# jafarinia/snuffy

Hardware: AMD Instinct MI355X
Metric: slides/sec (higher is better)
Workload: dtype f32; 1 GPU; cfgB: MILNet eval forward, 1 bag/step/rank, N=32768 patches D=768 h=6 Lambda=200 (K=200) depth=1 relu mlp x4; parallelism=bag-parallel x1, bags_resident_per_rank=8, launch=hip graph replay, rccl_ranks=0

## Files before the change

snuffy_amd/csrc/gemm.hip:

```cpp
#include <stdlib.h>

#include "mfma.h"
#include "philox.h"

namespace {

struct GemmParams {
    const unsigned short* a;
    const unsigned short* w;
    const float* bias;
    void* c;
    int64_t lda, ldw, ldc;
    int m, n, k;
    int act;
    int tiles_m, tiles_n;
    unsigned long long* trace;
    const float* resid = nullptr;
    int64_t ldr = 0;
    unsigned int* split_cnt = nullptr;
    float* split_slab = nullptr;
    int split_cap = 0, split_rcap = 0;
    const unsigned short* gate = nullptr;
    int64_t ldg = 0;
    const float* colsum = nullptr;
// ... 384 lines not shown
    for (int i = 0; i < AHEAD; ++i) stage(cur, i, i);
    wait_vmcnt<(AHEAD - 1) * GL>();
    __builtin_amdgcn_s_barrier();
    __builtin_amdgcn_sched_barrier(0);
    if (wid >= 4) __builtin_amdgcn_s_barrier();

    int rb = 0, sb = AHEAD;
    bool after_epilogue = false;
    while (true) {
        const int next = tile + wgs_per_xcd;
        const bool has_next = next < t_hi;
        const Src nxt = tile_src(has_next ? next : tile);
        const bool full = (tile / P.tiles_n + 1) * BM <= P.m && (tile % P.tiles_n + 1) * BN <= P.n;
        for (int s = 0; s < ns; ++s) {
            if constexpr (EPI == 2)
                if (s == 0) preload_x(tile);
            read_frags(rb);
            if (s == ns - 1) load_bias(tile);
            const bool in_tile = s + AHEAD < ns;
            const int exist = has_next ? AHEAD : (ns - 1 - s < AHEAD ? ns - 1 - s : AHEAD);
            if (in_tile)
                stage(cur, s + AHEAD, sb);
            else if (has_next)
                stage(nxt, s + AHEAD - ns, sb);
            if (exist == AHEAD) {
                if (after_epilogue)
                    wait_vmcnt<(AHEAD - 1) * GL + MI * NST>();
                else
                    wait_vmcnt<(AHEAD - 1) * GL>();
            } else if (AHEAD == 3 && exist == 2) {
                wait_vmcnt<GL>();
            } else {
                wait_vmcnt<0>();
            }
            after_epilogue = false;
            rb = rb == NBUF - 1 ? 0 : rb + 1;
            sb = sb == NBUF - 1 ? 0 : sb + 1;
            barrier();
            if (s == 0)
                mma(std::true_type{});
            else
                mma(std::false_type{});
            barrier();
        }
        bias_landed();
#ifdef SNF_GEMM_NOSTORE
        if (false) {
#else
        if (full) {
#endif
            epilogue(tile, std::true_type{});
            after_epilogue = true;
        } else {
            epilogue(tile, std::false_type{});
            wait_vmcnt<0>();
        }
        if (!has_next) break;
        tile = next;
        cur = nxt;
    }
    if (wid < 4) __builtin_amdgcn_s_barrier();
}

template <int ACT, int OUT, bool SPLIT = false, bool GATE = false, bool DROP = false>
__global__ __launch_bounds__(512, 2) void gemm_hl_kernel(GemmParams P) {
    static_assert(!GATE || (OUT == 3 && ACT == SNF_ACT_NONE && !SPLIT), "gemm_hl: the gated form writes an hl image, no activation, no split");
    static_assert(!DROP || (!GATE && (OUT == 1 || OUT == 3)), "gemm_hl: dropout goes with the fp32 and the hl-image outputs");
    constexpr int NI = 4, BN = 256;
    constexpr int ROWL = 128;
    constexpr int IMG = BM * ROWL;
    constexpr int STEP_BYTES = 2 * IMG;
    constexpr int NC = 4 * NI;
    constexpr bool LINE_STORES = (OUT == 1 || OUT == 3) && ACT != SNF_ACT_GELU && ACT != SNF_ACT_SELU;
    extern __shared__ __attribute__((aligned(16))) unsigned char smem[];

    const int lane = threadIdx.x & 63;
    const int wid = __builtin_amdgcn_readfirstlane(threadIdx.x >> 6);
    const int wr = wid >> 2, wc = wid & 3;
    const int ns_all = P.k / BKS;
    unsigned char* const scr = smem + 2 * STEP_BYTES + wid * 4096;

    const int ntiles = P.tiles_m * P.tiles_n;
    const int xcd = blockIdx.x & 7, wg_in_xcd = blockIdx.x >> 3, wgs_per_xcd = gridDim.x >> 3;
    if constexpr (!SPLIT) {
        if (P.split_cap >= 2 && blockIdx.x == 0) {
            for (int i = threadIdx.x; i < 8 * P.split_rcap; i += 512) P.split_cnt[i] = 0u;
            asm volatile("s_waitcnt vmcnt(0)" ::: "memory");
        }
    }
    int t_lo, t_hi;
    {
        const int q = ntiles >> 3, r = ntiles & 7;
        t_lo = xcd < r ? xcd * (q + 1) : r * (q + 1) + (xcd - r) * q;
        t_hi = t_lo + q + (xcd < r ? 1 : 0);
    }
    int sp_part = 0, sp_parts = 1, sp_slot = 0, sp_tile = -1;
    if (P.split_cap >= 2) {
        const int q_x = t_hi - t_lo, full_rounds = q_x / wgs_per_xcd, r = q_x - full_rounds * wgs_per_xcd;
        int sn = r > 0 ? wgs_per_xcd / r : 0;
        if (sn > P.split_cap) sn = P.split_cap;
        if (sn > ns_all / HL_SPLIT_MIN_STEPS) sn = ns_all / HL_SPLIT_MIN_STEPS;
        if (sn >= 2 && r <= P.split_rcap) {
            if constexpr (SPLIT) {
                if (wg_in_xcd < r * sn) {
                    const int jr = wg_in_xcd % r;
                    sp_tile = t_lo + full_rounds * wgs_per_xcd + jr;
                    sp_part = wg_in_xcd / r, sp_parts = sn, sp_slot = xcd * P.split_rcap + jr;
                }
            } else {
                t_hi = t_lo + full_rounds * wgs_per_xcd;
            }
        }
    }
    int tile = t_lo + wg_in_xcd;
    if constexpr (SPLIT) {
        tile = __builtin_amdgcn_readfirstlane(sp_tile);
        sp_part = __builtin_amdgcn_readfirstlane(sp_part), sp_parts = __builtin_amdgcn_readfirstlane(sp_parts);
        sp_slot = __builtin_amdgcn_readfirstlane(sp_slot);
        if (tile < 0) return;
        t_hi = tile + 1;
        asm volatile("" : "+s"(t_hi));
    } else {
        if (tile >= t_hi) return;
    }
    const int s_begin = SPLIT ? __builtin_amdgcn_readfirstlane(sp_part * ns_all / sp_parts) : 0;
    const int ns = SPLIT ? __builtin_amdgcn_readfirstlane((sp_part + 1) * ns_all / sp_parts) - s_begin : ns_all;
    const unsigned short* const a_base = P.a + (SPLIT ? s_begin * 64 : 0);
    const unsigned short* const w_base = P.w + (SPLIT ? s_begin * 64 : 0);

    struct Src {
        int a[4], w[4];
    };
    auto tile_src_mn = [&](int tm, int tn) __attribute__((always_inline)) -> Src {
        Src s;
        int ln = lane;
        asm volatile("" : "+v"(ln));
        const int c = ln & 7;
#pragma unroll
        for (int j = 0; j < 4; ++j) {
            const int row = (4 * wid + j) * 8 + (ln >> 3);
            int grow = tm * BM + row;
            if (grow > P.m - 1) grow = P.m - 1;
            s.a[j] = grow * (int)P.lda + ((c ^ ((row >> 1) & 7)) << 3);
            int wrow = tn * BN + row;
            if (wrow > P.n - 1) wrow = P.n - 1;
            s.w[j] = wrow * (int)P.ldw + ((c ^ (((row >> 1) & 1) | (((row >> 3) & 3) << 1))) << 3);
        }
        return s;
    };
    auto tile_src = [&](int tl) __attribute__((always_inline)) -> Src {
        const int tm = tl / P.tiles_n;
        return tile_src_mn(tm, tl - tm * P.tiles_n);
    };
    auto stage = [&](const Src& s, int kstep, int buf) __attribute__((always_inline)) {
#ifdef X3_NOSTAGE
        return;
#endif
        unsigned char* base = smem + buf * STEP_BYTES;
#pragma unroll
        for (int j = 0; j < 4; ++j) {
            __builtin_amdgcn_global_load_lds((glb_void*)(a_base + s.a[j] + kstep * 64), (lds_void*)(base + (4 * wid + j) * 1024), 16, 0, 0);
            __builtin_amdgcn_global_load_lds((glb_void*)(w_base + s.w[j] + kstep * 64), (lds_void*)(base + IMG + (4 * wid + j) * 1024), 16, 0, 0);
        }
    };

    const int fi = lane & 15, fg = lane >> 4;
    const int fa = (fi >> 1) & 7, fw = ((fi >> 1) & 1) | ((fi >> 2) << 1);
    const int xoff_h = (128 * wr + fi) * ROWL + ((fg ^ fa) << 4), xoff_l = (128 * wr + fi) * ROWL + (((4 + fg) ^ fa) << 4);
    const int wrow0 = IMG + (64 * wc + 8 * (fi >> 2) + (fi & 3)) * ROWL;
    const int woff_h = wrow0 + ((fg ^ fw) << 4), woff_l = wrow0 + (((4 + fg) ^ fw) << 4);

    f32x4 acc[8][NI];
    bf16x8 xf[8], wh[NI], wl[NI];
    f32x4 bv4[NC / 4];

    auto frag = [&](const unsigned char* p) __attribute__((always_inline)) -> bf16x8 {
#ifdef X3_NOREAD
        u32x4 z = {1u, 2u, 3u, (unsigned)lane};
        asm volatile("" : "+v"(z));
        return __builtin_bit_cast(bf16x8, z);
#endif
        return __builtin_bit_cast(bf16x8, *reinterpret_cast<const u32x4*>(p));
    };
#ifdef X3_NOMFMA
#define X3_MFMA(a, b, c) ([&]() { f32x4 t_ = (c); asm volatile("" : "+v"(t_) : "v"(a), "v"(b)); return t_; }())
#else
#define X3_MFMA(a, b, c) __builtin_amdgcn_mfma_f32_16x16x32_bf16(a, b, c, 0, 0, 0)
#endif
    auto load_bias = [&](int tl) __attribute__((always_inline)) {
#pragma unroll
        for (int c4 = 0; c4 < NC / 4; ++c4) bv4[c4] = f32x4{0.f, 0.f, 0.f, 0.f};
        if (P.bias) {
            const int tn = tl % P.tiles_n;
            const int n0 = tn * BN + 64 * wc + 8 * fg;
            const float* bp0 = P.bias + (n0 + 8 <= P.n ? n0 : 0);
            const float* bp1 = P.bias + (n0 + 40 <= P.n ? n0 + 32 : 0);
            asm volatile("global_load_dwordx4 %0, %1, off" : "=v"(bv4[0]) : "v"(bp0) : "memory");
            asm volatile("global_load_dwordx4 %0, %1, off offset:16" : "=v"(bv4[1]) : "v"(bp0) : "memory");
            asm volatile("global_load_dwordx4 %0, %1, off" : "=v"(bv4[2]) : "v"(bp1) : "memory");
            asm volatile("global_load_dwordx4 %0, %1, off offset:16" : "=v"(bv4[3]) : "v"(bp1) : "memory");
        }
    };
    auto bias_landed = [&]() __attribute__((always_inline)) {
#pragma unroll
        for (int c4 = 0; c4 < NC / 4; ++c4) asm volatile("" : "+v"(bv4[c4]));
    };
    auto epilogue = [&](int tl, auto full_t) __attribute__((always_inline)) {
        constexpr bool FULL = decltype(full_t)::value;
        const int tm = tl / P.tiles_n, tn = tl - tm * P.tiles_n;
        const int n0 = tn * BN + 64 * wc + 8 * fg;
        const int row0 = tm * BM + 128 * wr + fi;
// ... 17 lines not shown
                        v[e] *= m0[e];
                        v[4 + e] *= m1[e];
                    }
#pragma unroll
                    for (int e = 0; e < 8; ++e) asm volatile("" : "+v"(v[e]));
                }
#ifdef X3_NOSTORE
                const bool ok = v[0] == 123.456f;
#else
                const bool ok = FULL || (row < P.m && col + 8 <= P.n);
#endif
                if constexpr (GATE) {
                    u32x4 gv = {0u, 0u, 0u, 0u};
                    if (ok) gv = *reinterpret_cast<const u32x4*>(P.gate + (int64_t)row * P.ldg + 64 * (col >> 5) + (col & 31));
#pragma unroll
                    for (int e = 0; e < 4; ++e) {
                        if (!(__uint_as_float(gv[e] << 16) > 0.f)) v[2 * e] = 0.f;
                        if (!(__uint_as_float(gv[e] & 0xffff0000u) > 0.f)) v[2 * e + 1] = 0.f;
                    }
                }
                if constexpr (OUT == 1) {
                    float* dst = reinterpret_cast<float*>(P.c) + (int64_t)row * P.ldc + col;
                    if (P.resid && ok) {
                        const float* rp = P.resid + (int64_t)row * P.ldr + col;
                        const f32x4 r0 = *reinterpret_cast<const f32x4*>(rp), r1 = *reinterpret_cast<const f32x4*>(rp + 4);
#pragma unroll
                        for (int e = 0; e < 4; ++e) {
                            v[e] += r0[e];
                            v[4 + e] += r1[e];
                        }
                    }
                    if constexpr (LINE_STORES) {
                        *reinterpret_cast<f32x4*>(scr + fio * 256 + (((8 * h + 2 * fgo) ^ fio) << 4)) = f32x4{v[0], v[1], v[2], v[3]};
                        *reinterpret_cast<f32x4*>(scr + fio * 256 + (((8 * h + 2 * fgo + 1) ^ fio) << 4)) = f32x4{v[4], v[5], v[6], v[7]};
                    } else if (ok) {
                        *reinterpret_cast<f32x4*>(dst) = f32x4{v[0], v[1], v[2], v[3]};
                        *reinterpret_cast<f32x4*>(dst + 4) = f32x4{v[4], v[5], v[6], v[7]};
                    }
                } else {
                    const u32x4 pk = {cvt_pk_bf16(v[0], v[1]), cvt_pk_bf16(v[2], v[3]), cvt_pk_bf16(v[4], v[5]), cvt_pk_bf16(v[6], v[7])};
                    if constexpr (OUT == 0) {
                        unsigned short* dst = reinterpret_cast<unsigned short*>(P.c) + (int64_t)row * P.ldc + col;
                        if (ok) *reinterpret_cast<u32x4*>(dst) = pk;
                    } else {
                        float lo[8];
#pragma unroll
                        for (int e = 0; e < 8; ++e)
                            lo[e] = v[e] - __uint_as_float((e & 1) ? (pk[e >> 1] & 0xffff0000u) : (pk[e >> 1] << 16));
                        const u32x4 pl = {cvt_pk_bf16(lo[0], lo[1]), cvt_pk_bf16(lo[2], lo[3]), cvt_pk_bf16(lo[4], lo[5]), cvt_pk_bf16(lo[6], lo[7])};
                        unsigned short* dst = reinterpret_cast<unsigned short*>(P.c) + (int64_t)row * P.ldc + 64 * (col >> 5) + (col & 31);
                        if constexpr (LINE_STORES) {
                            *reinterpret_cast<u32x4*>(scr + fio * 256 + (((8 * h + fgo) ^ fio) << 4)) = pk;
                            *reinterpret_cast<u32x4*>(scr + fio * 256 + (((8 * h + 4 + fgo) ^ fio) << 4)) = pl;
                        } else if (ok) {
                            *reinterpret_cast<u32x4*>(dst) = pk;
                            *reinterpret_cast<u32x4*>(dst + 32) = pl;
                        }
                    }
                }
            }
            if constexpr (LINE_STORES) {
                const int lr = lane_o >> 4, lc = lane_o & 15;
                unsigned char* const crow = reinterpret_cast<unsigned char*>(P.c) +
                                            (OUT == 1 ? 4 * (int64_t)(tn * BN + 64 * wc) : 2 * 2 * (int64_t)(tn * BN + 64 * wc));
                const int64_t pitch = (OUT == 1 ? 4 : 2) * P.ldc;
#pragma unroll
                for (int jj = 0; jj < 4; ++jj) {
                    const int r = lr + 4 * jj;
                    const u32x4 val = *reinterpret_cast<const u32x4*>(scr + r * 256 + ((lc ^ r) << 4));
                    const int orow = tm * BM + 128 * wr + 16 * mi + r;
                    const int ocol = tn * BN + 64 * wc + (OUT == 1 ? 4 * lc : 32 * (lc >> 3) + 8 * (lc & 3));
#ifdef X3_NOSTORE
                    const bool ok2 = val[0] == 0x12345678u && orow < 0;
#else
                    const bool ok2 = FULL || (orow < P.m && ocol + (OUT == 1 ? 4 : 8) <= P.n);
#endif
                    if (ok2) *reinterpret_cast<u32x4*>(crow + orow * pitch + 16 * lc) = val;
                }
            }
        }
    };

    Src cur = tile_src(tile);
    stage(cur, 0, 0);
    int buf = 0;
    bool after_epilogue = false;
    while (true) {
        const int next = tile + wgs_per_xcd;
        const bool has_next = next < t_hi;
        const bool full = (tile / P.tiles_n + 1) * BM <= P.m && (tile % P.tiles_n + 1) * BN <= P.n;
        for (int s = 0; s < ns; ++s) {
            if (!(s == 0 && after_epilogue)) wait_vmcnt<0>();
            after_epilogue = false;
            __builtin_amdgcn_sched_barrier(0);
            __builtin_amdgcn_s_barrier();
            __builtin_amdgcn_sched_barrier(0);
            const unsigned char* base = smem + buf * STEP_BYTES;
#pragma unroll
            for (int ni = 0; ni < NI; ++ni) wh[ni] = frag(base + woff_h + (4 * (ni & 1) + 32 * (ni >> 1)) * ROWL);
#pragma unroll
            for (int mi = 0; mi < 8; ++mi) xf[mi] = frag(base + xoff_h + mi * 16 * ROWL);
#pragma unroll
            for (int ni = 0; ni < NI; ++ni) wl[ni] = frag(base + woff_l + (4 * (ni & 1) + 32 * (ni >> 1)) * ROWL);
            __builtin_amdgcn_sched_barrier(0);
            if (s + 1 < ns) {
                stage(cur, s + 1, buf ^ 1);
            } else if (has_next) {
                cur = tile_src(next);
                stage(cur, 0, buf ^ 1);
            }
            __builtin_amdgcn_sched_barrier(0);
            __builtin_amdgcn_s_setprio(1);
            if (s == 0) {
#pragma unroll
                for (int mi = 0; mi < 8; ++mi)
#pragma unroll
                    for (int ni = 0; ni < NI; ++ni) acc[mi][ni] = X3_MFMA(wh[ni], xf[mi], (f32x4{0.f, 0.f, 0.f, 0.f}));
            } else {
#pragma unroll
                for (int mi = 0; mi < 8; ++mi)
#pragma unroll
                    for (int ni = 0; ni < NI; ++ni) acc[mi][ni] = X3_MFMA(wh[ni], xf[mi], acc[mi][ni]);
            }
#pragma unroll
            for (int mi = 0; mi < 8; ++mi) {
#pragma unroll
                for (int ni = 0; ni < NI; ++ni) acc[mi][ni] = X3_MFMA(wl[ni], xf[mi], acc[mi][ni]);
                __builtin_amdgcn_sched_barrier(0);
                xf[mi] = frag(base + xoff_l + mi * 16 * ROWL);
                __builtin_amdgcn_sched_barrier(0);
            }
#pragma unroll
            for (int mi = 0; mi < 8; ++mi)
#pragma unroll
                for (int ni = 0; ni < NI; ++ni) acc[mi][ni] = X3_MFMA(wh[ni], xf[mi], acc[mi][ni]);
            __builtin_amdgcn_s_setprio(0);
            buf ^= 1;
        }
        if constexpr (SPLIT) {
            volatile unsigned int& s_ticket = *reinterpret_cast<volatile unsigned int*>(smem);
            float* slab0 = P.split_slab + (size_t)sp_slot * P.split_cap * (size_t)(BM * BN);
            unsigned tix = threadIdx.x;
            asm volatile("" : "+v"(tix));
            f32x4* mine = reinterpret_cast<f32x4*>(slab0 + (size_t)sp_part * (BM * BN)) + tix;
            wait_vmcnt<0>();
#pragma unroll
            for (int mi = 0; mi < 8; ++mi)
#pragma unroll
                for (int ni = 0; ni < NI; ++ni) mine[(mi * NI + ni) * 512] = acc[mi][ni];
            wait_vmcnt<0>();
            __syncthreads();
            if (tix == 0) {
                __builtin_amdgcn_fence(__ATOMIC_RELEASE, "agent");
                asm volatile("s_waitcnt vmcnt(0)" ::: "memory");
                s_ticket = __hip_atomic_fetch_add(P.split_cnt + sp_slot, 1u, __ATOMIC_RELAXED, __HIP_MEMORY_SCOPE_AGENT);
            }
            __syncthreads();
            if (s_ticket != (unsigned)(sp_parts - 1)) return;
            __syncthreads();
            if (tix == 0) {
                __builtin_amdgcn_fence(__ATOMIC_ACQUIRE, "agent");
                __hip_atomic_store(P.split_cnt + sp_slot, 0u, __ATOMIC_RELAXED, __HIP_MEMORY_SCOPE_AGENT);
            }
            __syncthreads();
#pragma unroll
            for (int mi = 0; mi < 8; ++mi)
#pragma unroll
                for (int ni = 0; ni < NI; ++ni) {
                    f32x4 sum = {0.f, 0.f, 0.f, 0.f};
                    for (int pp = 0; pp < sp_parts; ++pp) {
                        f32x4 v = acc[mi][ni];
                        if (pp != sp_part) v = reinterpret_cast<const f32x4*>(slab0 + (size_t)pp * (BM * BN))[(mi * NI + ni) * 512 + tix];
                        sum = pp == 0 ? v : sum + v;
                    }
                    acc[mi][ni] = sum;
                }
        }
        load_bias(tile);
        wait_vmcnt<0>();
        bias_landed();
        if (full)
            epilogue(tile, std::true_type{});
        else
            epilogue(tile, std::false_type{});
        after_epilogue = true;
        if (!has_next) break;
        tile = next;
    }
}

template <int ACT, int OUT, bool DROP = false>
int launch_hl(const GemmParams& P, hipStream_t s) {
    constexpr int lds = 2 * 2 * BM * 128 + (((OUT == 1 || OUT == 3) && ACT != SNF_ACT_GELU && ACT != SNF_ACT_SELU) ? 8 * 4096 : 0);
    auto kern = [] {
        if constexpr (DROP) return gemm_hl_kernel<ACT, OUT, false, false, true>;
        else return gemm_hl_kernel<ACT, OUT>;
    }();
    static thread_local unsigned long long attr_set_mask = 0;
    if (int rc = snf::lds_opt_in(reinterpret_cast<const void*>(kern), lds, &attr_set_mask, "gemm_hl")) return rc;
    const int ntiles = P.tiles_m * P.tiles_n;
    int grid = snf::cu_count() & ~7;
    if (grid < 8) grid = 8;
    {
        static const int dbg_grid = getenv("SNF_GEMM_HL_GRID") ? atoi(getenv("SNF_GEMM_HL_GRID")) & ~7 : 0;
        if (dbg_grid >= 8 && dbg_grid < grid && P.split_cap < 2) grid = dbg_grid;
    }
    const int per_xcd = (ntiles + 7) / 8;
    if (per_xcd * 8 < grid) grid = per_xcd * 8;
    hipLaunchKernelGGL(kern, dim3(grid), dim3(512), lds, s, P);
    int rc = snf::check_launch("gemm_hl_kernel");
    if (rc || P.split_cap < 2) return rc;
    auto kern2 = [] {
        if constexpr (DROP) return gemm_hl_kernel<ACT, OUT, true, false, true>;
        else return gemm_hl_kernel<ACT, OUT, true>;
    }();
    static thread_local unsigned long long attr_set2_mask = 0;
    if (int rc = snf::lds_opt_in(reinterpret_cast<const void*>(kern2), lds, &attr_set2_mask, "gemm_hl")) return rc;
    hipLaunchKernelGGL(kern2, dim3(grid), dim3(512), lds, s, P);
    return snf::check_launch("gemm_hl_kernel<split>");
}

int launch_hl_gated(const GemmParams& P, hipStream_t s) {
    constexpr int lds = 2 * 2 * BM * 128 + 8 * 4096;
    auto kern = gemm_hl_kernel<SNF_ACT_NONE, 3, false, true>;
    static thread_local unsigned long long attr_set_mask = 0;
    if (int rc = snf::lds_opt_in(reinterpret_cast<const void*>(kern), lds, &attr_set_mask, "gemm_hl")) return rc;
    const int ntiles = P.tiles_m * P.tiles_n;
    int grid = snf::cu_count() & ~7;
    if (grid < 8) grid = 8;
    const int per_xcd = (ntiles + 7) / 8;
    if (per_xcd * 8 < grid) grid = per_xcd * 8;
    hipLaunchKernelGGL(kern, dim3(grid), dim3(512), lds, s, P);
    return snf::check_launch("gemm_hl_kernel<gated>");
}

template <int OUT>
int launch_hl_act(const GemmParams& P, hipStream_t s) {
    switch (P.act) {
        case SNF_ACT_RELU: return launch_hl<SNF_ACT_RELU, OUT>(P, s);
        case SNF_ACT_GELU: return launch_hl<SNF_ACT_GELU, OUT>(P, s);
        case SNF_ACT_LEAKYRELU: return launch_hl<SNF_ACT_LEAKYRELU, OUT>(P, s);
        case SNF_ACT_SELU: return launch_hl<SNF_ACT_SELU, OUT>(P, s);
        default: return launch_hl<SNF_ACT_NONE, OUT>(P, s);
    }
}

template <int NI, int ACT, int OUT, int EPI = 0, int MI = 8>
int launch(const GemmParams& P, hipStream_t s) {
    constexpr int lds = NBUF * (A_BYTES + (MI == 8 ? 64 : 32) * NI * ROWB) +
                        ((EPI == 2 || (OUT == 0 && NI == 4 && ACT != SNF_ACT_GELU && ACT != SNF_ACT_SELU)) ? 8 * 4096 : 0);
    auto kern = gemm_bf16_kernel<NI, ACT, OUT, EPI, MI>;
    static thread_local unsigned long long attr_set_mask = 0;
    if (int rc = snf::lds_opt_in(reinterpret_cast<const void*>(kern), lds, &attr_set_mask, "gemm_bf16")) return rc;
    const int ntiles = P.tiles_m * P.tiles_n;
    int grid = snf::cu_count() & ~7;
    if (grid < 8) grid = 8;
    const int per_xcd = (ntiles + 7) / 8;
    if (per_xcd * 8 < grid) grid = per_xcd * 8;
    hipLaunchKernelGGL(kern, dim3(grid), dim3(512), lds, s, P);
    return snf::check_launch("gemm_bf16_kernel");
}

#ifndef SNF_GEMM_128_MI4
#define SNF_GEMM_128_MI4 1
#endif
template <int NI, int ACT, int OUT, int EPI = 0>
int launch_tile(const GemmParams& P, hipStream_t s) {
    if constexpr (NI == 2 && SNF_GEMM_128_MI4)
        return launch<4, ACT, OUT, EPI, 4>(P, s);
    else
        return launch<NI, ACT, OUT, EPI>(P, s);
}

template <int NI, int OUT>
int launch_act(const GemmParams& P, hipStream_t s) {
    switch (P.act) {
        case SNF_ACT_RELU: return launch_tile<NI, SNF_ACT_RELU, OUT>(P, s);
        case SNF_ACT_GELU: return launch_tile<NI, SNF_ACT_GELU, OUT>(P, s);
        case SNF_ACT_LEAKYRELU: return launch_tile<NI, SNF_ACT_LEAKYRELU, OUT>(P, s);
        case SNF_ACT_SELU: return launch_tile<NI, SNF_ACT_SELU, OUT>(P, s);
        default: return launch_tile<NI, SNF_ACT_NONE, OUT>(P, s);
    }
}

struct SkinnyFrag {
    int dk, chunk_size;
    int64_t chunk_stride;
    float c_exp;
    const int64_t* idx = nullptr;
    int64_t n_rows = 0;
    float* xs = nullptr;
    int64_t ldxs = 0;
    int32_t* map = nullptr;
    const float* resid = nullptr;
    float* out2 = nullptr;
    int64_t ldr = 0, ldo2 = 0;
};
template <bool OUT_BF16, bool FRAG = false>
__global__ __launch_bounds__(512) void skinny_linear_x3_kernel(const float* __restrict__ x, int64_t ldx, const float* __restrict__ w,
                                                                int64_t ldw, const float* __restrict__ bias, int r, int c, int k,
                                                                void* __restrict__ out, int64_t ldo, SkinnyFrag fr = SkinnyFrag{}) {
    constexpr int NW = 8, BATCH = 6;
// ... 449 lines not shown
```

snuffy_amd/ops.py:

```python
import ctypes
import math

import torch

from . import _ffi
from ._ffi import ACT_CODES, DT_BF16, DT_BF16_HL, DT_BF16_SPLIT3, DT_F32, TOPK_MAX_K, check


def _p(t):
    return None if t is None else ctypes.c_void_p(t.data_ptr())


_raw_stream = getattr(torch._C, "_cuda_getCurrentRawStream", None)


def _stream():
    if _raw_stream is not None:
        return ctypes.c_void_p(_raw_stream(torch.cuda.current_device()))
    return ctypes.c_void_p(torch.cuda.current_stream().cuda_stream)


def _on_current_device(t, name):
    if t.device.index != torch.cuda.current_device():
        raise _ffi.SnuffyHipError("%s lives on %s but the current device is cuda:%d: select the tensor's device first "
                                  "(torch.cuda.set_device / torch.cuda.device)" % (name, t.device, torch.cuda.current_device()))


def _req(t, dtype, name, dim=None):
    if not isinstance(t, torch.Tensor) or not t.is_cuda:
        raise _ffi.SnuffyHipError(
            "%s must be a GPU tensor: snuffy_amd runs on MI355X only (no CPU fallback)" % name)
    _on_current_device(t, name)
    if t.dtype != dtype:
        raise TypeError("%s must be %s, got %s" % (name, dtype, t.dtype))
    if dim is not None and t.dim() != dim:
        raise ValueError("%s must be %d-D, got shape %s" % (name, dim, tuple(t.shape)))
    return t if t.is_contiguous() else t.contiguous()


def _ws(nbytes, device):
    return torch.empty(max(int(nbytes), 16), dtype=torch.uint8, device=device)


def critic(x, w, b=None, want_max=False):
    x = _req(x, torch.float32, "x", 2)
    w = _req(w, torch.float32, "w", 2)
    if b is not None:
        b = _req(b, torch.float32, "b", 1)
    n, d = x.shape
    c = w.shape[0]
    if w.shape[1] != d:
        raise ValueError("critic: w is %s but x has %d features" % (tuple(w.shape), d))
    scores = torch.empty(n, c, dtype=torch.float32, device=x.device)
    mv = mi = None
    if want_max:
        mv = torch.empty(c, dtype=torch.float32, device=x.device)
        mi = torch.empty(c, dtype=torch.int64, device=x.device)
    check(_ffi.load().snf_critic_f32(_p(x), n, d, _p(w), _p(b), c, _p(scores), _p(mv), _p(mi), _stream()),
          "snf_critic_f32")
    return (scores, mv, mi) if want_max else scores


def critic_ln(x, w, b, eps):
    x = _req(x, torch.float32, "x", 2)
    w = _req(w, torch.float32, "w", 2)
    if b is not None:
        b = _req(b, torch.float32, "b", 1)
    n, d = x.shape
    c = w.shape[0]
    if w.shape[1] != d:
        raise ValueError("critic_ln: w is %s but x has %d features" % (tuple(w.shape), d))
    scores = torch.empty(n, c, dtype=torch.float32, device=x.device)
    xhat = torch.empty(n, d, dtype=torch.bfloat16, device=x.device)
    check(_ffi.load().snf_critic_ln_f32(_p(x), n, d, _p(w), _p(b), c, _p(scores), float(eps), _p(xhat), _stream()),
          "snf_critic_ln_f32")
    return scores, xhat


SELECT_FUSED_MIN_N = 16385
_SELECTORS = {}


class _Selector:
    def __init__(self, device):
        lib = _ffi.load()
        self.nbytes = int(lib.snf_selector_state_bytes())
        self.state = torch.zeros(self.nbytes, dtype=torch.uint8, device=device)
        self.pending = None


def _selector_key(device):
    raw = _raw_stream(device.index) if _raw_stream is not None else torch.cuda.current_stream(device).cuda_stream
    return (device.index, int(raw))


def selector(device, create=True):
    key = _selector_key(device)
    sel = _SELECTORS.get(key)
    if sel is None and create and not torch.cuda.is_current_stream_capturing():
        sel = _SELECTORS[key] = _Selector(device)
    return sel


def fresh_selector(device):
    sel = _SELECTORS[_selector_key(device)] = _Selector(device)
    return sel


def critic_select(x, w, b, eps=None):
    if w.shape[0] != 1 or x.shape[0] < SELECT_FUSED_MIN_N or x.shape[0] >= (1 << 30):
        return None
    sel = selector(x.device)
    if sel is None:
        return None
    x = _req(x, torch.float32, "x", 2)
    w = _req(w, torch.float32, "w", 2)
    if b is not None:
        b = _req(b, torch.float32, "b", 1)
    n, d = x.shape
    if w.shape[1] != d:
        raise ValueError("critic_select: w is %s but x has %d features" % (tuple(w.shape), d))
    if sel.pending is not None:
        sel.state.zero_()
        sel.pending = None
    scores = torch.empty(n, 1, dtype=torch.float32, device=x.device)
    xhat = torch.empty(n, d, dtype=torch.bfloat16, device=x.device) if eps is not None else None
    check(_ffi.load().snf_critic_select_f32(_p(x), n, d, _p(w), _p(b), _p(scores), float(eps or 0.0), _p(xhat), _p(sel.state),
                                            _stream()), "snf_critic_select_f32")
    sel.pending = (scores.data_ptr(), n, scores._version)
    return scores, xhat


def critic_ln_hl(x, w, b, gamma, beta, eps):
    x = _req(x, torch.float32, "x", 2)
    w = _req(w, torch.float32, "w", 2)
    if b is not None:
        b = _req(b, torch.float32, "b", 1)
    if (gamma is None) != (beta is None):
        raise ValueError("critic_ln_hl: gamma and beta: both or neither (neither = the affine-free image)")
    if gamma is not None:
        gamma = _req(gamma, torch.float32, "gamma", 1)
        beta = _req(beta, torch.float32, "beta", 1)
    n, d = x.shape
    c = w.shape[0]
    if w.shape[1] != d or d % 32:
        raise ValueError("critic_ln_hl: w is %s, x has %d features (need d %% 32 == 0)" % (tuple(w.shape), d))
    sel = selector(x.device) if (c == 1 and SELECT_FUSED_MIN_N <= n < (1 << 30)) else None
    if sel is not None and sel.pending is not None:
        sel.state.zero_()
        sel.pending = None
    scores = torch.empty(n, c, dtype=torch.float32, device=x.device)
    img = torch.empty(n, 2 * d, dtype=torch.bfloat16, device=x.device)
    check(_ffi.load().snf_critic_ln_hl_f32(_p(x), n, d, _p(w), _p(b), c, _p(scores), _p(gamma), _p(beta), float(eps), _p(img),
                                           _p(sel.state) if sel is not None else None, _stream()), "snf_critic_ln_hl_f32")
    if sel is not None:
        sel.pending = (scores.data_ptr(), n, scores._version)
    return scores, img


def topk(scores, k, x=None):
    if not scores.is_cuda:
        raise _ffi.SnuffyHipError("topk: scores must be a GPU tensor (no CPU fallback)")
    if scores.dtype != torch.float32 or scores.dim() != 1:
        raise TypeError("topk: scores must be 1-D float32")
    n = scores.shape[0]
    stride = scores.stride(0) if n > 1 else 1
    if stride < 1:
        scores = scores.contiguous()
        stride = 1
    k = int(k)
    if not (1 <= k <= n):
# ... 1088 lines not shown
        if out is None:
            out = torch.empty(m, n, dtype=out_dtype, device=a_hl.device)
        odt = DT_F32 if out.dtype == torch.float32 else DT_BF16
    ldr = 0
    if resid is not None:
        if hl_out or out.dtype != torch.float32 or resid.dtype != torch.float32 or tuple(resid.shape) != (m, n):
            raise ValueError("gemm_hl: resid needs an fp32 [m, n] tensor and an fp32 output")
        resid = _rows16(resid, "resid")
        ldr = resid.stride(0)
    lib = _ffi.load()
    ws, ws_bytes = None, 0
    if GEMM_HL_SPLITK:
        ws_bytes = int(lib.snf_gemm_hl_ws_bytes(m, n, k2 // 2))
        if ws_bytes:
            ws = _hl_workspace(a_hl.device, ws_bytes)
    check(lib.snf_gemm_hl_ws_bf16(_p(a_hl), a_hl.stride(0), _p(w_hl), w_hl.stride(0), _p(bias), _p(resid), ldr, m, n, k2 // 2,
                                  ACT_CODES[act], _p(out), out.stride(0), odt, _p(ws), ws_bytes, _stream()), "snf_gemm_hl_ws_bf16")
    return out


def encoder_dropout_supported(n, d, f):
    return d % 32 == 0 and f % 32 == 0 and d <= 8192 and hl_eligible(n, f, d) and hl_eligible(n, d, f)


def gemm_hl_dropout(a_hl, w_hl, bias, dropout, act="none", hl_out=False, resid=None, out=None):
    if a_hl.dtype != torch.bfloat16 or w_hl.dtype != torch.bfloat16:
        raise TypeError("gemm_hl_dropout: operands must be bfloat16 hl images")
    if (act, bool(hl_out)) not in (("relu", True), ("none", False)):
        raise ValueError("gemm_hl_dropout: only relu -> hl image and none -> fp32 (+ resid) exist")
    a_hl = _rows16(a_hl, "a_hl")
    w_hl = _rows16(w_hl, "w_hl")
    m, k2 = a_hl.shape
    n = w_hl.shape[0]
    if w_hl.shape[1] != k2 or k2 % 64 or (hl_out and n % 32):
        raise ValueError("gemm_hl_dropout: images are %s and %s" % (tuple(a_hl.shape), tuple(w_hl.shape)))
    if bias is not None:
        bias = _req(bias, torch.float32, "bias", 1)
    if out is None:
        out = torch.empty(m, 2 * n, dtype=torch.bfloat16, device=a_hl.device) if hl_out else \
            torch.empty(m, n, dtype=torch.float32, device=a_hl.device)
    odt = DT_BF16_HL if hl_out else DT_F32
    ldr = 0
    if resid is not None:
        if hl_out or resid.dtype != torch.float32 or tuple(resid.shape) != (m, n):
            raise ValueError("gemm_hl_dropout: resid needs an fp32 [m, n] tensor and an fp32 output")
        resid = _rows16(resid, "resid")
        ldr = resid.stride(0)
    p, seed, offset = dropout
    lib = _ffi.load()
    ws, ws_bytes = None, 0
    if GEMM_HL_SPLITK:
        ws_bytes = int(lib.snf_gemm_hl_ws_bytes(m, n, k2 // 2))
        if ws_bytes:
            ws = _hl_workspace(a_hl.device, ws_bytes)
    check(lib.snf_gemm_hl_ws_dropout_bf16(_p(a_hl), a_hl.stride(0), _p(w_hl), w_hl.stride(0), _p(bias), _p(resid), ldr, m, n, k2 // 2,
                                          ACT_CODES[act], _p(out), out.stride(0), odt, float(p), int(seed) & (2 ** 64 - 1),
                                          int(offset) & (2 ** 64 - 1), _p(ws), ws_bytes, _stream()), "snf_gemm_hl_ws_dropout_bf16")
    return out


def gemm_hl_gated(a_hl, w_hl, gate_hl):
    a_hl, w_hl, gate_hl = _rows16(a_hl, "a_hl"), _rows16(w_hl, "w_hl"), _rows16(gate_hl, "gate_hl")
    if a_hl.dtype != torch.bfloat16 or w_hl.dtype != torch.bfloat16 or gate_hl.dtype != torch.bfloat16:
        raise TypeError("gemm_hl_gated: operands must be bfloat16 hl images")
    m, k2 = a_hl.shape
    n = w_hl.shape[0]
    if w_hl.shape[1] != k2 or k2 % 64 or n % 32 or tuple(gate_hl.shape) != (m, 2 * n):
        raise ValueError("gemm_hl_gated: inconsistent shapes")
    out = torch.empty(m, 2 * n, dtype=torch.bfloat16, device=a_hl.device)
    check(_ffi.load().snf_gemm_hl_gated_bf16(_p(a_hl), a_hl.stride(0), _p(w_hl), w_hl.stride(0), _p(gate_hl), gate_hl.stride(0), m, n,
                                             k2 // 2, _p(out), out.stride(0), _stream()), "snf_gemm_hl_gated_bf16")
    return out


def hl_colsum(img):
    s, _ = colsum_fused(img)
    return s.view(-1, 2, 32).sum(1).reshape(-1)


GEMM_HL_SPLITK = True


def _hl_workspace(device, nbytes):
    return _ws(nbytes, device)


def split3_weight(w, colscale=None):
    w = w.detach().float()
    if colscale is not None:
        colscale = colscale.detach().float().contiguous()
    if w.is_cuda and w.dim() == 2 and w.shape[1] % 8 == 0 and w.stride(1) == 1 and w.stride(0) % 4 == 0 and w.data_ptr() % 16 == 0:
        out = torch.empty(w.shape[0], 3 * w.shape[1], dtype=torch.bfloat16, device=w.device)
        check(_ffi.load().snf_split3_weight_f32(_p(w), w.stride(0), w.shape[0], w.shape[1], _p(colscale), _p(out), _stream()),
              "snf_split3_weight_f32")
        return out
    if colscale is not None:
        w = w * colscale
    hi = w.to(torch.bfloat16)
    lo = (w - hi.float()).to(torch.bfloat16)
    return torch.cat([hi, lo, hi], dim=1).contiguous()


def split3_rows(x):
    if x.dtype != torch.float32:
        raise TypeError("split3_rows: x must be float32")
    x = _rows16(x, "x")
    m, k = x.shape
    if k % 8:
        hi = x.to(torch.bfloat16)
        lo = (x - hi.float()).to(torch.bfloat16)
        return torch.cat([hi, hi, lo], dim=1).contiguous()
    out = torch.empty(m, 3 * k, dtype=torch.bfloat16, device=x.device)
    check(_ffi.load().snf_split3_f32(_p(x), x.stride(0), m, k, _p(out), _stream()), "snf_split3_f32")
    return out


def split3_colsum(x, gate=None, out=None, col=0, want_colsum=True):
    if x.dtype != torch.float32:
        raise TypeError("split3_colsum: x must be float32")
    x = _rows16(x, "x")
    m, k = x.shape
    if k % 8 or k > 8192:
        raise ValueError("split3_colsum: k=%d must be a multiple of 8 and <= 8192" % k)
    ldg = 0
    if gate is not None:
        if gate.dtype != torch.bfloat16 or tuple(gate.shape) != (m, k):
            raise ValueError("split3_colsum: gate must be bfloat16 of the shape of x")
        gate = _rows16(gate, "gate")
        ldg = gate.stride(0)
    if out is None:
        out = torch.empty(m, 3 * k, dtype=torch.bfloat16, device=x.device)
        col = 0
    elif (out.dtype != torch.bfloat16 or out.dim() != 2 or not out.is_contiguous() or out.shape[0] != m or out.shape[1] % 3
          or col % 8 or col + k > out.shape[1] // 3):
        raise ValueError("split3_colsum: bad out image")
    plane = out.shape[1] // 3
    lib = _ffi.load()
    part = torch.empty(lib.snf_colsum_blocks(m), k, dtype=torch.float32, device=x.device) if want_colsum else None
    dst = out if col == 0 else out[:, col:]
    check(lib.snf_split3_colsum_f32(_p(x), x.stride(0), m, k, _p(gate), ldg, _p(dst), out.stride(0), plane, _p(part), _stream()),
          "snf_split3_colsum_f32")
    return out, (part.sum(0) if part is not None else None)


def split_hl_colsum(x, gate_hl=None, out=None, col=0, want_colsum=True, dropout=None):
    if x.dtype != torch.float32:
        raise TypeError("split_hl_colsum: x must be float32")
    x = _rows16(x, "x")
    m, k = x.shape
    if k % 32 or k > 8192:
        raise ValueError("split_hl_colsum: k=%d must be a multiple of 32 and <= 8192" % k)
    ldg = 0
    if gate_hl is not None:
        if gate_hl.dtype != torch.bfloat16 or tuple(gate_hl.shape) != (m, 2 * k):
            raise ValueError("split_hl_colsum: gate must be the bfloat16 hl image of a matrix of the shape of x")
        gate_hl = _rows16(gate_hl, "gate")
        ldg = gate_hl.stride(0)
    if out is None:
        out = torch.empty(m, 2 * k, dtype=torch.bfloat16, device=x.device)
        col = 0
    elif (out.dtype != torch.bfloat16 or out.dim() != 2 or not out.is_contiguous() or out.shape[0] != m or out.shape[1] % 64
          or col % 32 or 2 * (col + k) > out.shape[1]):
        raise ValueError("split_hl_colsum: bad out image")
    lib = _ffi.load()
    part = torch.empty(lib.snf_colsum_blocks(m), k, dtype=torch.float32, device=x.device) if want_colsum else None
    dst = out if col == 0 else out[:, 2 * col:]
    if dropout is not None:
# ... 149 lines not shown
```

Baseline: 870.5 slides/s.

## Fuse split-K tail tiles into the main GEMM launch instead of a second kernel

The split-K GEMM path now runs as a single kernel. Workgroups first process their full tiles and then pick up a K-slice of a leftover tail tile, where before a second split kernel was launched after the main one. Partial sums go through the slab with an atomic ticket, and the last arriving part reduces them and runs the epilogue. The in-kernel zeroing of the counters by block 0 is dropped; instead a persistent per-selector workspace is zeroed once on the host side and the kernel resets each counter after use. This removes one kernel launch and the tail-wave gap, at the cost of more complex control flow and reliance on counters being left clean between calls.

```diff
diff --git a/snuffy_amd/csrc/gemm.hip b/snuffy_amd/csrc/gemm.hip
--- a/snuffy_amd/csrc/gemm.hip
+++ b/snuffy_amd/csrc/gemm.hip
@@ -490,51 +490,46 @@
 
     const int ntiles = P.tiles_m * P.tiles_n;
     const int xcd = blockIdx.x & 7, wg_in_xcd = blockIdx.x >> 3, wgs_per_xcd = gridDim.x >> 3;
-    if constexpr (!SPLIT) {
-        if (P.split_cap >= 2 && blockIdx.x == 0) {
-            for (int i = threadIdx.x; i < 8 * P.split_rcap; i += 512) P.split_cnt[i] = 0u;
-            asm volatile("s_waitcnt vmcnt(0)" ::: "memory");
-        }
-    }
     int t_lo, t_hi;
     {
         const int q = ntiles >> 3, r = ntiles & 7;
         t_lo = xcd < r ? xcd * (q + 1) : r * (q + 1) + (xcd - r) * q;
         t_hi = t_lo + q + (xcd < r ? 1 : 0);
     }
-    int sp_part = 0, sp_parts = 1, sp_slot = 0, sp_tile = -1;
-    if (P.split_cap >= 2) {
+    int sp_part = 0, sp_parts = 1, sp_slot = 0, sp_tile = -1, sp_begin = 0, sp_ns = 0;
+    if constexpr (SPLIT) {
         const int q_x = t_hi - t_lo, full_rounds = q_x / wgs_per_xcd, r = q_x - full_rounds * wgs_per_xcd;
         int sn = r > 0 ? wgs_per_xcd / r : 0;
         if (sn > P.split_cap) sn = P.split_cap;
         if (sn > ns_all / HL_SPLIT_MIN_STEPS) sn = ns_all / HL_SPLIT_MIN_STEPS;
         if (sn >= 2 && r <= P.split_rcap) {
-            if constexpr (SPLIT) {
-                if (wg_in_xcd < r * sn) {
-                    const int jr = wg_in_xcd % r;
-                    sp_tile = t_lo + full_rounds * wgs_per_xcd + jr;
-                    sp_part = wg_in_xcd / r, sp_parts = sn, sp_slot = xcd * P.split_rcap + jr;
-                }
-            } else {
-                t_hi = t_lo + full_rounds * wgs_per_xcd;
-            }
-        }
-    }
-    int tile = t_lo + wg_in_xcd;
-    if constexpr (SPLIT) {
-        tile = __builtin_amdgcn_readfirstlane(sp_tile);
+            t_hi = t_lo + full_rounds * wgs_per_xcd;
+            if (wg_in_xcd < r * sn) {
+                const int jr = wg_in_xcd % r;
+                sp_tile = t_lo + full_rounds * wgs_per_xcd + jr;
+                sp_part = wg_in_xcd / r, sp_parts = sn, sp_slot = xcd * P.split_rcap + jr;
+                sp_begin = sp_part * ns_all / sp_parts;
+                sp_ns = (sp_part + 1) * ns_all / sp_parts - sp_begin;
+            }
+        }
+        t_hi = __builtin_amdgcn_readfirstlane(t_hi), sp_tile = __builtin_amdgcn_readfirstlane(sp_tile);
         sp_part = __builtin_amdgcn_readfirstlane(sp_part), sp_parts = __builtin_amdgcn_readfirstlane(sp_parts);
         sp_slot = __builtin_amdgcn_readfirstlane(sp_slot);
-        if (tile < 0) return;
-        t_hi = tile + 1;
-        asm volatile("" : "+s"(t_hi));
+        sp_begin = __builtin_amdgcn_readfirstlane(sp_begin), sp_ns = __builtin_amdgcn_readfirstlane(sp_ns);
+    }
+    int tile = t_lo + wg_in_xcd;
+    bool part = false;
+    if constexpr (SPLIT) {
+        if (sp_tile >= 0 && (sp_part > 0 || tile >= t_hi)) {
+            tile = sp_tile, part = true;
+        } else if (tile >= t_hi) {
+            return;
+        }
     } else {
         if (tile >= t_hi) return;
     }
-    const int s_begin = SPLIT ? __builtin_amdgcn_readfirstlane(sp_part * ns_all / sp_parts) : 0;
-    const int ns = SPLIT ? __builtin_amdgcn_readfirstlane((sp_part + 1) * ns_all / sp_parts) - s_begin : ns_all;
-    const unsigned short* const a_base = P.a + (SPLIT ? s_begin * 64 : 0);
-    const unsigned short* const w_base = P.w + (SPLIT ? s_begin * 64 : 0);
+    const unsigned short* const a_base = P.a;
+    const unsigned short* const w_base = P.w;
 
     struct Src {
         int a[4], w[4];
@@ -718,12 +713,22 @@
     };
 
     Src cur = tile_src(tile);
-    stage(cur, 0, 0);
+    stage(cur, SPLIT && part ? sp_begin : 0, 0);
     int buf = 0;
     bool after_epilogue = false;
     while (true) {
-        const int next = tile + wgs_per_xcd;
-        const bool has_next = next < t_hi;
+        int next = tile + wgs_per_xcd;
+        bool has_next = next < t_hi, next_part = false;
+        if constexpr (SPLIT) {
+            if (part) {
+                next = t_lo + wg_in_xcd;
+                has_next = sp_part > 0 && next < t_hi;
+            } else if (!has_next && sp_tile >= 0 && sp_part == 0) {
+                next = sp_tile, has_next = true, next_part = true;
+            }
+        }
+        const int s_begin = SPLIT && part ? sp_begin : 0;
+        const int ns = SPLIT && part ? sp_ns : ns_all;
         const bool full = (tile / P.tiles_n + 1) * BM <= P.m && (tile % P.tiles_n + 1) * BN <= P.n;
         for (int s = 0; s < ns; ++s) {
             if (!(s == 0 && after_epilogue)) wait_vmcnt<0>();
@@ -740,7 +745,7 @@
             for (int ni = 0; ni < NI; ++ni) wl[ni] = frag(base + woff_l + (4 * (ni & 1) + 32 * (ni >> 1)) * ROWL);
             __builtin_amdgcn_sched_barrier(0);
             if (s + 1 < ns) {
-                stage(cur, s + 1, buf ^ 1);
+                stage(cur, s_begin + s + 1, buf ^ 1);
             } else if (has_next) {
                 cur = tile_src(next);
                 stage(cur, 0, buf ^ 1);
@@ -773,65 +778,77 @@
             __builtin_amdgcn_s_setprio(0);
             buf ^= 1;
         }
+        bool parked = false;
         if constexpr (SPLIT) {
-            volatile unsigned int& s_ticket = *reinterpret_cast<volatile unsigned int*>(smem);
-            float* slab0 = P.split_slab + (size_t)sp_slot * P.split_cap * (size_t)(BM * BN);
-            unsigned tix = threadIdx.x;
-            asm volatile("" : "+v"(tix));
-            f32x4* mine = reinterpret_cast<f32x4*>(slab0 + (size_t)sp_part * (BM * BN)) + tix;
+            if (part) {
+                volatile unsigned int& s_ticket = *reinterpret_cast<volatile unsigned int*>(smem + (buf ^ 1) * STEP_BYTES);
+                float* slab0 = P.split_slab + (size_t)sp_slot * P.split_cap * (size_t)(BM * BN);
+                unsigned tix = threadIdx.x;
+                asm volatile("" : "+v"(tix));
+                __syncthreads();
+                if (tix == 0) s_ticket = __hip_atomic_load(P.split_cnt + sp_slot, __ATOMIC_RELAXED, __HIP_MEMORY_SCOPE_AGENT);
+                __syncthreads();
+                bool last = s_ticket == (unsigned)(sp_parts - 1);
+                if (!last) {
+                    f32x4* mine = reinterpret_cast<f32x4*>(slab0 + (size_t)sp_part * (BM * BN)) + tix;
+#pragma unroll
+                    for (int mi = 0; mi < 8; ++mi)
+#pragma unroll
+                        for (int ni = 0; ni < NI; ++ni) mine[(mi * NI + ni) * 512] = acc[mi][ni];
+                    wait_vmcnt<0>();
+                    __syncthreads();
+                    if (tix == 0) {
+                        __builtin_amdgcn_fence(__ATOMIC_RELEASE, "agent");
+                        asm volatile("s_waitcnt vmcnt(0)" ::: "memory");
+                        s_ticket = __hip_atomic_fetch_add(P.split_cnt + sp_slot, 1u, __ATOMIC_RELAXED, __HIP_MEMORY_SCOPE_AGENT);
+                    }
+                    __syncthreads();
+                    last = s_ticket == (unsigned)(sp_parts - 1);
+                }
+                if (last) {
+                    __syncthreads();
+                    if (tix == 0) {
+                        __builtin_amdgcn_fence(__ATOMIC_ACQUIRE, "agent");
+                        __hip_atomic_store(P.split_cnt + sp_slot, 0u, __ATOMIC_RELAXED, __HIP_MEMORY_SCOPE_AGENT);
+                    }
+                    __syncthreads();
+#pragma unroll
+                    for (int mi = 0; mi < 8; ++mi)
+#pragma unroll
+                        for (int ni = 0; ni < NI; ++ni) {
+                            f32x4 sum = {0.f, 0.f, 0.f, 0.f};
+                            for (int pp = 0; pp < sp_parts; ++pp) {
+                                f32x4 v = acc[mi][ni];
+                                if (pp != sp_part) v = reinterpret_cast<const f32x4*>(slab0 + (size_t)pp * (BM * BN))[(mi * NI + ni) * 512 + tix];
+                                sum = pp == 0 ? v : sum + v;
+                            }
+                            acc[mi][ni] = sum;
+                        }
+                } else {
+                    parked = true;
+                }
+            }
+        }
+        if (!parked) {
+            load_bias(tile);
             wait_vmcnt<0>();
-#pragma unroll
-            for (int mi = 0; mi < 8; ++mi)
-#pragma unroll
-                for (int ni = 0; ni < NI; ++ni) mine[(mi * NI + ni) * 512] = acc[mi][ni];
-            wait_vmcnt<0>();
-            __syncthreads();
-            if (tix == 0) {
-                __builtin_amdgcn_fence(__ATOMIC_RELEASE, "agent");
-                asm volatile("s_waitcnt vmcnt(0)" ::: "memory");
-                s_ticket = __hip_atomic_fetch_add(P.split_cnt + sp_slot, 1u, __ATOMIC_RELAXED, __HIP_MEMORY_SCOPE_AGENT);
-            }
-            __syncthreads();
-            if (s_ticket != (unsigned)(sp_parts - 1)) return;
-            __syncthreads();
-            if (tix == 0) {
-                __builtin_amdgcn_fence(__ATOMIC_ACQUIRE, "agent");
-                __hip_atomic_store(P.split_cnt + sp_slot, 0u, __ATOMIC_RELAXED, __HIP_MEMORY_SCOPE_AGENT);
-            }
-            __syncthreads();
-#pragma unroll
-            for (int mi = 0; mi < 8; ++mi)
-#pragma unroll
-                for (int ni = 0; ni < NI; ++ni) {
-                    f32x4 sum = {0.f, 0.f, 0.f, 0.f};
-                    for (int pp = 0; pp < sp_parts; ++pp) {
-                        f32x4 v = acc[mi][ni];
-                        if (pp != sp_part) v = reinterpret_cast<const f32x4*>(slab0 + (size_t)pp * (BM * BN))[(mi * NI + ni) * 512 + tix];
-                        sum = pp == 0 ? v : sum + v;
-                    }
-                    acc[mi][ni] = sum;
-                }
-        }
-        load_bias(tile);
-        wait_vmcnt<0>();
-        bias_landed();
-        if (full)
-            epilogue(tile, std::true_type{});
-        else
-            epilogue(tile, std::false_type{});
-        after_epilogue = true;
+            bias_landed();
+            if (full)
+                epilogue(tile, std::true_type{});
+            else
+                epilogue(tile, std::false_type{});
+            after_epilogue = true;
+        }
         if (!has_next) break;
         tile = next;
-    }
-}
-
-template <int ACT, int OUT, bool DROP = false>
-int launch_hl(const GemmParams& P, hipStream_t s) {
+        part = next_part;
+    }
+}
+
+template <int ACT, int OUT, bool DROP, bool SPLIT>
+int launch_hl_form(const GemmParams& P, hipStream_t s) {
     constexpr int lds = 2 * 2 * BM * 128 + (((OUT == 1 || OUT == 3) && ACT != SNF_ACT_GELU && ACT != SNF_ACT_SELU) ? 8 * 4096 : 0);
-    auto kern = [] {
-        if constexpr (DROP) return gemm_hl_kernel<ACT, OUT, false, false, true>;
-        else return gemm_hl_kernel<ACT, OUT>;
-    }();
+    auto kern = gemm_hl_kernel<ACT, OUT, SPLIT, false, DROP>;
     static thread_local unsigned long long attr_set_mask = 0;
     if (int rc = snf::lds_opt_in(reinterpret_cast<const void*>(kern), lds, &attr_set_mask, "gemm_hl")) return rc;
     const int ntiles = P.tiles_m * P.tiles_n;
@@ -839,21 +856,17 @@
     if (grid < 8) grid = 8;
     {
         static const int dbg_grid = getenv("SNF_GEMM_HL_GRID") ? atoi(getenv("SNF_GEMM_HL_GRID")) & ~7 : 0;
-        if (dbg_grid >= 8 && dbg_grid < grid && P.split_cap < 2) grid = dbg_grid;
+        if (dbg_grid >= 8 && dbg_grid < grid && !SPLIT) grid = dbg_grid;
     }
     const int per_xcd = (ntiles + 7) / 8;
     if (per_xcd * 8 < grid) grid = per_xcd * 8;
     hipLaunchKernelGGL(kern, dim3(grid), dim3(512), lds, s, P);
-    int rc = snf::check_launch("gemm_hl_kernel");
-    if (rc || P.split_cap < 2) return rc;
-    auto kern2 = [] {
-        if constexpr (DROP) return gemm_hl_kernel<ACT, OUT, true, false, true>;
-        else return gemm_hl_kernel<ACT, OUT, true>;
-    }();
-    static thread_local unsigned long long attr_set2_mask = 0;
-    if (int rc = snf::lds_opt_in(reinterpret_cast<const void*>(kern2), lds, &attr_set2_mask, "gemm_hl")) return rc;
-    hipLaunchKernelGGL(kern2, dim3(grid), dim3(512), lds, s, P);
-    return snf::check_launch("gemm_hl_kernel<split>");
+    return snf::check_launch(SPLIT ? "gemm_hl_kernel<split>" : "gemm_hl_kernel");
+}
+
+template <int ACT, int OUT, bool DROP = false>
+int launch_hl(const GemmParams& P, hipStream_t s) {
+    return P.split_cap >= 2 ? launch_hl_form<ACT, OUT, DROP, true>(P, s) : launch_hl_form<ACT, OUT, DROP, false>(P, s);
 }
 
 int launch_hl_gated(const GemmParams& P, hipStream_t s) {
diff --git a/snuffy_amd/ops.py b/snuffy_amd/ops.py
--- a/snuffy_amd/ops.py
+++ b/snuffy_amd/ops.py
@@ -87,6 +87,7 @@
         self.nbytes = int(lib.snf_selector_state_bytes())
         self.state = torch.zeros(self.nbytes, dtype=torch.uint8, device=device)
         self.pending = None
+        self.hl_ws = {}
 
 
 def _selector_key(device):
@@ -1341,7 +1342,16 @@
 
 
 def _hl_workspace(device, nbytes):
-    return _ws(nbytes, device)
+    sel = selector(device)
+    if sel is None:
+        ws = _ws(nbytes, device)
+        ws[:4096].zero_()
+        return ws
+    ws = sel.hl_ws.get(nbytes)
+    if ws is None:
+        ws = sel.hl_ws[nbytes] = torch.empty(nbytes, dtype=torch.uint8, device=device)
+        ws[:4096].zero_()
+    return ws
 
 
 def split3_weight(w, colscale=None):
```

Result: no change. 876.7 slides/s (median of 6 runs) (+0.7%).
